# iqbal-lab-org/make_prg

Hardware: AMD Instinct MI355X
Metric: MSAs/sec (from_msa, whole node) on 30k-gene pan-genome (higher is better)
Workload: dtype u8 (+f64 KMeans)

## Files before the change

make_prg_amd/csrc/k_partition.inc:

```
MPRG_DEV bool col_is_nonmatch(const uint32_t *mask, int c) { return consensus_code(mask[c]) == 255; }

#define GR_ROWS 256
#ifndef GR_SEG
#define GR_SEG 512
#endif
#ifndef GR_BATCH
#define GR_BATCH 16
#endif
MPRG_DEV long long gr_items(long long S, long long n) { return ((S + GR_ROWS - 1) / GR_ROWS) * ((n + GR_SEG - 1) / GR_SEG); }
KERNEL(k_gap_runs, const uint8_t *arena, const int64_t *views, const int32_t *rowidx, const int32_t *work,
       const uint32_t *mask_all, uint32_t *maxrun_all, DsCount dc) {
  DS_GUARD(dc, 1);
  const int32_t *wk = work + 2 * (long long)BLOCK_ID;
  const ViewD d = load_view(views, wk[0]);
  const int n_chunks = (d.n_rows + GR_ROWS - 1) / GR_ROWS;
  const int r0 = (wk[1] % n_chunks) * GR_ROWS, cA = (wk[1] / n_chunks) * GR_SEG, cB = cA + GR_SEG < d.n_cols ? cA + GR_SEG : d.n_cols;
  const uint32_t *mask = mask_all + d.col_off;
  uint32_t *maxrun = maxrun_all + d.col_off;
  SHARED(int, has_gap, 1);
  ONE_THREAD { has_gap[0] = 0; }
  BARRIER();
  PAR_FOR(c, cB - cA) { if (mask[cA + c] & BIT_GAP) has_gap[0] = 1; }
  BARRIER();
  if (!has_gap[0]) return;
// ... 223 lines not shown
    int status = 0, cnt = 0, expect = 0, im = 0, in = 0;
    const int pure = (sh[4] || sh[5]) ? 0 : 2;
    while (im < nm || in < nn) {
      const bool takeM = in >= nn || (im < nm && Ms[2 * im] <= Ns[2 * in]);
      int s, e, type;
      if (takeM) { s = Ms[2 * im]; e = Ms[2 * im + 1]; type = pure; ++im; }
      else {
        s = Ns[2 * in]; e = Ns[2 * in + 1];
        const int ty = FAST ? ntype_s[in] : NTYPE(in);
        if (ty == 3) status |= 2;
        type = ty & 1;
        ++in;
      }
      if (s != expect || e < s || e >= n) { status |= 1; break; }
      ivw[3 * cnt] = s; ivw[3 * cnt + 1] = e; ivw[3 * cnt + 2] = type;
      ++cnt;
      expect = e + 1;
    }
    if (expect != n || cnt != nm + nn) status |= 1;
    sh[6] = cnt; sh[3] = status; sh[7] = cnt > 0 ? (ivw[2] & 1) : 0;
  }
  P_BAR(); KM_T(20);
#undef PUSH_M
#undef PUSH_N
#undef NONMATCH
#undef NTYPE
#undef PCELL
#undef PCELL8
#undef P_FOR
#undef P_BAR
#undef P_ONE
}

template <bool WV = false>
MPRG_DEV void pt_outputs(int v, int *sh, bool fast, const uint8_t *nmz_s, int32_t *iv, int32_t *n_iv_out, int32_t *status_out,
                         int32_t *view_out KM_TPARAM) {
  if ((WV ? wave_lane() : MPRG_TID) == 0) {
    const int cnt = sh[6], status = sh[3];
    n_iv_out[v] = cnt;
    status_out[v] = status;
    if (view_out) {
      int32_t *o = view_out + 8 * (long long)v;
      o[0] = cnt; o[1] = status; o[2] = sh[7];
      o[3] = (sh[0] ? 1 : 0) | ((sh[4] || sh[5]) ? 2 : 0);
      o[4] = 0; o[5] = 0; o[6] = 0; o[7] = 0;
    }
  }
  KM_T(22);
  if (fast) {
    const int32_t *src = (const int32_t *)nmz_s;
    for (int e = WV ? wave_lane() : MPRG_TID; e < 3 * sh[6]; e += WV ? WAVE : (int)blockDim.x) iv[e] = src[e];
  }
}
#define PK_PER_THREAD 32
KERNEL(k_pack_scan, int n_views_cap, const int32_t *n_iv, int32_t *view_out, int32_t *iv_count, DsCount dc) {
  const int n_views = (int)ds_n(dc, n_views_cap);
  SHARED(int, scratch, 17);
  int base = 0;
  for (int v0 = 0; v0 < n_views; v0 += N_THREADS * PK_PER_THREAD) {
    const int v = v0 + (int)threadIdx.x * PK_PER_THREAD;
    int c[PK_PER_THREAD], sum = 0;
#pragma unroll
    for (int q = 0; q < PK_PER_THREAD; ++q) { c[q] = v + q < n_views ? n_iv[v + q] : 0; sum += c[q]; }
    int tot;
    int run = base + block_scan_excl(sum, scratch, &tot);
#pragma unroll
    for (int q = 0; q < PK_PER_THREAD; ++q) { if (v + q < n_views) view_out[8 * (long long)(v + q) + 4] = run; run += c[q]; }
    base += tot;
  }
  ONE_THREAD { iv_count[0] = base; }
}
#define PK_THREADS 256
KERNEL(k_pack_copy, int n_views, const int64_t *views, const int32_t *iv_all, const int32_t *view_out, int32_t *iv_packed, DsCount dc) {
  const int v = BLOCK_ID * (PK_THREADS / WAVE) + wave_id();
  if (v >= ds_n(dc, n_views)) return;
  const int32_t *o = view_out + 8 * (long long)v;
  const int32_t *src = iv_all + 3 * views[(long long)v * VF + 8];
  int32_t *dst = iv_packed + 3 * (long long)o[4];
  for (int e = wave_lane(); e < 3 * o[0]; e += WAVE) dst[e] = src[e];
}

KERNEL(k_partition, const int32_t *view_list, const uint8_t *arena, const int64_t *views, const int32_t *rowidx,
       const uint32_t *mask_all, int L, uint32_t *maxrun_all, int32_t *stack_all, int32_t *ivflag_all, int32_t *iv_all,
       int32_t *n_iv_out, int32_t *status_out, int32_t *view_out, DsCount dc) {
  DS_GUARD(dc, 1);
  KM_T0();
  const int v = view_list ? view_list[BLOCK_ID] : BLOCK_ID;
  const ViewD d = load_view(views, v);
  const int n = d.n_cols;
  const uint32_t *mask = mask_all + d.col_off;
  uint32_t *maxrun = maxrun_all + d.col_off;
  SHARED(int32_t, stk_s, 4 * PT_STACK);
  __shared__ __attribute__((aligned(16))) uint8_t nmz_s[PT_COLS];
  SHARED(int32_t, ntype_s, PT_STACK);
  const bool fast = n / (L > 1 ? L - 1 : 1) + 4 <= PT_STACK && n <= PT_COLS;
  int32_t *flag_multi = ivflag_all + 2 * d.col_off;
  int32_t *ref_row = flag_multi + n;
  int32_t *iv = iv_all + 3 * d.col_off;
  SHARED(int, sh, 8);
  ONE_THREAD { sh[0] = 0; sh[1] = 0; sh[2] = 0; sh[3] = 0; sh[4] = 0; sh[5] = 0; sh[6] = 0; sh[7] = 0; }
  BARRIER();
  PAR_FOR(c, n) {
    const uint32_t m = mask[c];
    if (m & BIT_N) sh[4] = 1;
    if (m & BITS_IUPAC) sh[5] = 1;
    const uint32_t mm = m & ~BIT_N;
    const bool star = !(mm != 0 && (mm & (mm - 1)) == 0 && (mm & BITS_IUPAC) == 0 && mm != BIT_GAP);
    if (star) sh[0] = 1;
    if (fast) nmz_s[c] = star ? 1 : 0;
  }
  BARRIER(); KM_T(16);
  if (fast) pt_phases<true, false>(arena, d, rowidx, mask, L, maxrun, stack_all + 4 * d.col_off, flag_multi, ref_row, iv, stk_s,
                                   PT_STACK, nmz_s, PT_COLS, ntype_s, sh, nullptr, 0 KM_TARG);
  else pt_phases<false, false>(arena, d, rowidx, mask, L, maxrun, stack_all + 4 * d.col_off, flag_multi, ref_row, iv, stk_s,
                               PT_STACK, nmz_s, PT_COLS, ntype_s, sh, nullptr, 0 KM_TARG);
  pt_outputs(v, sh, fast, nmz_s, iv, n_iv_out, status_out, view_out KM_TARG);
  KM_T(21);
}

#define PF_ROWS 512
#define PF_COLS 1024
#define PF_CELLS 8192
#define PF_STACK 128
// ... 190 lines not shown
```

make_prg_amd/csrc/k_rows.inc:

```
MPRG_DEV uint64_t hash_mix(uint64_t x) {
  x ^= x >> 30; x *= 0xbf58476d1ce4e5b9ULL; x ^= x >> 27; x *= 0x94d049bb133111ebULL; x ^= x >> 31;
  return x;
}
#ifdef MPRG_TEST_WEAK_HASH
#define MPRG_HASH_MIX(x) 1ULL
#else
#define MPRG_HASH_MIX(x) hash_mix(x)
#endif
MPRG_DEV int u_pitch(int n_cols) { return (n_cols + 15) & ~15; }
MPRG_DEV uint64_t wave_sum_u64(uint64_t v) {
#pragma unroll
  for (int d = 32; d >= 1; d >>= 1) v += (uint64_t)__shfl_xor((unsigned long long)v, d);
  return v;
}

#define UG_ROWS 256
#define UG_WIDE 4096
#define UG_ROWS_WIDE 8
#define UG_BATCH 4
MPRG_DEV int ug_chunk_rows(long long n_cols) { return n_cols > UG_WIDE ? UG_ROWS_WIDE : UG_ROWS; }
MPRG_DEV long long ug_chunks(long long S, long long n_cols) { const int ch = ug_chunk_rows(n_cols); return (S + ch - 1) / ch; }
MPRG_DEV uint64_t hash_word(uint64_t w, unsigned pos) { return MPRG_HASH_MIX(w ^ ((uint64_t)(pos + 1) << 40)); }
#define DW_WAVES 4
#define DW_ROWS 64
#define DW_SLOTS 128
#define DW_COLS 64
MPRG_DEV bool dw_is_small(long long S, long long n) { return S >= 1 && S <= DW_ROWS && n >= 1 && n <= DW_COLS; }
MPRG_DEV void ug_hash_rows(const uint8_t *arena, const ViewD &d, const int32_t *rowidx, int r0, int chunk, int wv, int n_waves,
                           uint8_t *ucodes_all, uint64_t *hashes, int32_t *ulen_all, uint8_t *gcodes_all) {
  const int n = d.n_cols, S = d.n_rows;
  const int upitch = u_pitch(n);
  uint8_t *U = ucodes_all + d.aux0;
  uint64_t *hg = hashes + 2 * d.row_off + S;
  int32_t *ulen = ulen_all + d.row_off;
  const int lane = wave_lane();
  int G = WAVE;
  while (G > 8 && 4 * (G >> 1) >= n) G >>= 1;
  const int rows_per_wave = WAVE / G, gl = lane & (G - 1), sub = lane / G;
  for (int ib = r0 + wv * rows_per_wave; ib < r0 + chunk && ib < S; ib += n_waves * rows_per_wave) {
    const int i = ib + sub;
    const bool live = i < S && i < r0 + chunk;
    const uint8_t *src = arena + d.rm + (long long)(live ? view_row(d, rowidx, i) : 0) * d.pitchC + d.col0;
    uint8_t *dst = U + (long long)i * upitch;
    uint8_t *gdst = gcodes_all ? gcodes_all + d.aux0 + (long long)i * upitch : nullptr;
    uint64_t g = 0;
    int len = 0;
#define UG_STEP(w_, c0_) do {                                                                                                          \
      const int c = (c0_) + 4 * gl;                                                                                                    \
      uint32_t w = (w_);                                                                                                               \
      if (live && c < n) {                                                                                                             \
        if (c + 4 > n) {                                                          \
          const uint32_t keep = 0xffffffffu >> (8 * (c + 4 - n));                                                                      \
          w = (w & keep) | (0x04040404u & ~keep);                                                                                      \
        }                                                                                                                              \
        g += hash_word(w, (unsigned)c);                                                                                                \
        if (gdst) __builtin_memcpy(gdst + c, &w, 4);                        \
      }                                                                                                                                \
      const uint32_t v = w ^ 0x04040404u;                                                                       \
      const uint32_t gap = ~(((v & 0x7f7f7f7fu) + 0x7f7f7f7fu) | v) & 0x80808080u;                \
      const int kept = 4 - __popc(gap);                                                                                                \
      int incl = kept;                                                                \
      for (int dd = 1; dd < G; dd <<= 1) { const int y = __shfl_up(incl, dd, G); if (gl >= dd) incl += y; }                            \
      const int at = len + incl - kept;                                                                                                \
      if (live) {                                                                                                                      \
        if (kept == 4) __builtin_memcpy(dst + at, &w, 4);                                                                              \
        else if (kept) {                                                                                                               \
          int o = at;                                                                                                                  \
          _Pragma("unroll") for (int u = 0; u < 4; ++u) if (!((gap >> (8 * u + 7)) & 1u)) dst[o++] = (uint8_t)(w >> (8 * u));        \
        }                                                                                                                              \
      }                                                                                                                                \
      len += __shfl(incl, G - 1, G);                                                                                                   \
    } while (0)
    if (n <= 4 * G) {
      uint32_t w0 = 0x04040404u;
      if (live && 4 * gl < n) __builtin_memcpy(&w0, src + 4 * gl, 4);
      UG_STEP(w0, 0);
    } else {
      for (int cb = 0; cb < n; cb += UG_BATCH * 4 * G) {
        uint32_t wq[UG_BATCH];
#pragma unroll
        for (int q = 0; q < UG_BATCH; ++q) {
          const int c = cb + q * 4 * G + 4 * gl;
          wq[q] = 0x04040404u;
          if (live && c < n) __builtin_memcpy(&wq[q], src + c, 4);
        }
#pragma unroll
        for (int q = 0; q < UG_BATCH; ++q) {
          if (cb + q * 4 * G >= n) break;
          UG_STEP(wq[q], cb + q * 4 * G);
        }
      }
    }
#undef UG_STEP
    for (int dd = G >> 1; dd >= 1; dd >>= 1) g += (uint64_t)__shfl_xor((unsigned long long)g, dd, G);
    if (live && gl == 0) { hg[i] = g; ulen[i] = len; }
  }
}
KERNEL(k_ungap_hash, const uint8_t *arena, const int64_t *views, const int32_t *rowidx, const int32_t *work,
       uint8_t *ucodes_all, uint64_t *hashes, int32_t *ulen_all, uint8_t *gcodes_all, int wave_form, DsCount dc) {
  DS_GUARD(dc, 1);
  const int32_t *wk = work + 2 * (long long)BLOCK_ID;
  const ViewD d = load_view(views, wk[0]);
  if (wave_form && dw_is_small(d.n_rows, d.n_cols)) return;
  const int chunk = ug_chunk_rows(d.n_cols);
  ug_hash_rows(arena, d, rowidx, wk[1] * chunk, chunk, wave_id(), N_THREADS / WAVE, ucodes_all, hashes, ulen_all, gcodes_all);
}

MPRG_DEV void ug_hash_u_rows(const ViewD &d, int r0, int chunk, int wv, int n_waves, const uint8_t *ucodes_all, uint64_t *hashes,
                             const int32_t *ulen_all) {
  const int n = d.n_cols, S = d.n_rows, upitch = u_pitch(n);
  const uint8_t *U = ucodes_all + d.aux0;
  uint64_t *hu_w = hashes + 2 * d.row_off;
  const int32_t *ulen = ulen_all + d.row_off;
  const int lane = wave_lane();
  int G = WAVE;
  while (G > 4 && 8 * (G >> 1) >= n) G >>= 1;
  const int rows_per_wave = WAVE / G, gl = lane & (G - 1), sub = lane / G;
  for (int ib = r0 + wv * rows_per_wave; ib < r0 + chunk && ib < S; ib += n_waves * rows_per_wave) {
    const int i = ib + sub;
    const bool live = i < S && i < r0 + chunk;
    const int len = live ? ulen[i] : 0;
    const uint8_t *row = U + (long long)(live ? i : 0) * upitch;
    uint64_t a = 0;
    for (int p = 8 * gl; p < len; p += 8 * G) {
      uint64_t w = *(const uint64_t *)(row + p);
      if (p + 8 > len) w &= 0xffffffffffffffffULL >> (8 * (p + 8 - len));
      a += hash_word(w, (unsigned)p);
    }
    for (int dd = G >> 1; dd >= 1; dd >>= 1) a += (uint64_t)__shfl_xor((unsigned long long)a, dd, G);
    if (live && gl == 0) hu_w[i] = a;
  }
}
KERNEL(k_ungap_hash_u, const int64_t *views, const int32_t *work, const uint8_t *ucodes_all, uint64_t *hashes, const int32_t *ulen_all,
       int wave_form, DsCount dc) {
  DS_GUARD(dc, 1);
  const int32_t *wk = work + 2 * (long long)BLOCK_ID;
  const ViewD d = load_view(views, wk[0]);
  if (wave_form && dw_is_small(d.n_rows, d.n_cols)) return;
  const int chunk = ug_chunk_rows(d.n_cols);
  ug_hash_u_rows(d, wk[1] * chunk, chunk, wave_id(), N_THREADS / WAVE, ucodes_all, hashes, ulen_all);
}

#define DD_ROWS 512
#define DD_SLOTS 1024
#define DD_EMPTY 0xffffffffffffffffULL
MPRG_DEV bool dd_diff_u16(const uint8_t *U, int upitch, int i, int j, int p0, int len) {
  const uint4 x = *(const uint4 *)(U + (long long)i * upitch + p0), y = *(const uint4 *)(U + (long long)j * upitch + p0);
  unsigned m[4] = {x.x ^ y.x, x.y ^ y.y, x.z ^ y.z, x.w ^ y.w};
  const int valid = len - p0;
  if (valid >= 16) return (m[0] | m[1] | m[2] | m[3]) != 0;
  unsigned bad = 0;
#pragma unroll
  for (int w = 0; w < 4; ++w) {
    const int vb = valid - 4 * w;
    const unsigned keep = vb >= 4 ? 0xffffffffu : (vb <= 0 ? 0u : ((1u << (8 * vb)) - 1u));
    bad |= m[w] & keep;
  }
  return bad != 0;
}
KERNEL(k_dedupe_scan_big, const uint8_t *arena, const int64_t *views, const int32_t *rowidx, const int32_t *work,
       const uint8_t *ucodes_all, const uint64_t *hashes, const int32_t *ulen_all, int32_t *rep_u_all, int32_t *rep_g_all, DsCount dc) {
  DS_GUARD(dc, 1);
  const int32_t *wk = work + 2 * (long long)BLOCK_ID;
  const ViewD d = load_view(views, wk[0]);
  const int n = d.n_cols, S = d.n_rows, chunk = ug_chunk_rows(n), r0 = wk[1] * chunk, upitch = u_pitch(n);
  if (S <= DD_ROWS) return;
  const uint8_t *U = ucodes_all + d.aux0;
  const uint64_t *hu = hashes + 2 * d.row_off, *hg = hu + S;
  const int32_t *ulen = ulen_all + d.row_off;
  __shared__ uint64_t s_hu[DD_ROWS], s_hg[DD_ROWS];
  __shared__ int32_t s_len[DD_ROWS];
  __shared__ int32_t s_ru[UG_ROWS], s_rg[UG_ROWS];
  const int i_end = r0 + chunk < S ? r0 + chunk : S;
  const int G = N_THREADS / chunk > 0 ? N_THREADS / chunk : 1, ri_ = (int)threadIdx.x % chunk, cls = (int)threadIdx.x / chunk;
  const int i = r0 + ri_;
  const bool live = cls < G && i < i_end;
  if (threadIdx.x < UG_ROWS) { s_ru[threadIdx.x] = 0x7fffffff; s_rg[threadIdx.x] = 0x7fffffff; }
  const uint64_t a = live ? hu[i] : 0, g = live ? hg[i] : 0;
  const int len = live ? ulen[i] : 0;
  const uint8_t *ri = arena + d.rm + (long long)(live ? view_row(d, rowidx, i) : 0) * d.pitchC + d.col0;
  for (int c0 = 0; c0 < i_end - 1; c0 += DD_ROWS) {
    BARRIER();
    const bool done_u = s_ru[ri_] != 0x7fffffff, done_g = s_rg[ri_] != 0x7fffffff;
    PAR_FOR(t, DD_ROWS) { if (c0 + t < S) { s_hu[t] = hu[c0 + t]; s_hg[t] = hg[c0 + t]; s_len[t] = ulen[c0 + t]; } }
    BARRIER();
    if (!live || i <= c0) continue;
    const int j1 = (i < c0 + DD_ROWS ? i : c0 + DD_ROWS) - c0;
    if (!done_u) {
      for (int t0 = cls; t0 < j1;) {
        int hit = 0x7fffffff;
        for (int t = t0; t < j1 && hit == 0x7fffffff; t += 8 * G) {
#pragma unroll
          for (int q = 7; q >= 0; --q) { const int tq = t + q * G; if (tq < j1 && s_hu[tq] == a && s_len[tq] == len) hit = tq; }
        }
        if (hit == 0x7fffffff) break;
        bool bad = false;
        for (int p = 0; p < len && !bad; p += 16) bad = dd_diff_u16(U, upitch, i, c0 + hit, p, len);
// ... 13 lines not shown
        bool bad = false;
        for (int c = 0; c < n && !bad; ++c) bad = ri[c] != rj[c];
        if (!bad) { atomicMin(&s_rg[ri_], c0 + hit); break; }
        t0 = hit + G;
      }
    }
  }
  BARRIER();
  if (live && cls == 0) {
    rep_u_all[d.row_off + i] = s_ru[ri_] == 0x7fffffff ? i : s_ru[ri_];
    rep_g_all[d.row_off + i] = s_rg[ri_] == 0x7fffffff ? i : s_rg[ri_];
  }
}

#define DD_EXACT(HU, HG, LEN, RU, RG)                                                                                   \
  P_FOR(i, S) {                                                                                                       \
    int ru = (int)i;                                                                                                    \
    const int len = LEN[i];                                                                                             \
    const uint64_t a = HU[i];                                                                                           \
    for (int j = 0; j < (int)i; ++j) {                                                                                  \
      if (HU[j] != a || LEN[j] != len) continue;                                                                        \
      bool bad = false;                                                                                                 \
      for (int p = 0; p < len && !bad; p += 16) bad = dd_diff_u16(U, upitch, (int)i, j, p, len);                        \
      if (!bad) { ru = j; break; }                                                                                      \
    }                                                                                                                   \
    int rg = (int)i;                                                                                                    \
    const uint64_t g = HG[i];                                                                                           \
    const uint8_t *ri = arena + d.rm + (long long)view_row(d, rowidx, i) * d.pitchC + d.col0;                           \
    for (int j = 0; j < (int)i; ++j) {                                                                                  \
      if (HG[j] != g) continue;                                                                                         \
      const uint8_t *rj = arena + d.rm + (long long)view_row(d, rowidx, j) * d.pitchC + d.col0;                         \
      bool bad = false;                                                                                                 \
      for (int c = 0; c < n && !bad; ++c) bad = ri[c] != rj[c];                                                         \
      if (!bad) { rg = j; break; }                                                                                      \
    }                                                                                                                   \
    RU[i] = ru; RG[i] = rg;                                                                                             \
  }

template <int ROWS, int SLOTS> struct DdLds {
  unsigned long long t_key[SLOTS];
  uint64_t s_hu[ROWS], s_hg[ROWS];
  int t_min[SLOTS];
  int32_t s_len[ROWS], s_ru[ROWS], s_rg[ROWS];
  long long wsum[16];
  int scan_tmp[17];
  int refuted[1];
};
template <bool WV> MPRG_DEV int dd_scan_excl(int v, int *scratch, int *total) {
  if (!WV) return block_scan_excl(v, scratch, total);
  const int incl = wave_scan_incl(v);
  *total = __shfl(incl, WAVE - 1);
  return incl - v;
}
template <bool WV, int ROWS, int SLOTS>
MPRG_DEV void dd_view(const int q, const ViewD &d, const uint8_t *arena, const int32_t *rowidx, int kmer_size,
                      uint8_t *ucodes_all, const uint8_t *gcodes_all, uint64_t *hashes, int32_t *ulen_all, int32_t *rep_u_all, int32_t *rep_g_all,
                      int32_t *d_of_row_all, int32_t *s_of_row_all, int32_t *reps_pos_all, int32_t *reps_len_all,
                      int32_t *seqrow_all, int64_t *occ_off_all, int64_t *summary, DdLds<ROWS, SLOTS> &L) {
#define P_FOR(i_, n_) for (long long i_ = WV ? wave_lane() : MPRG_TID; i_ < (long long)(n_); i_ += WV ? WAVE : (int)blockDim.x)
#define P_BAR() do { if (WV) WAVE_SYNC(); else BARRIER(); } while (0)
#define P_ONE if ((WV ? wave_lane() : MPRG_TID) == 0)
  const int n = d.n_cols, S = d.n_rows;
  const int upitch = u_pitch(n);
  const uint8_t *U = ucodes_all + d.aux0;
  const uint64_t *hu = hashes + 2 * d.row_off, *hg = hu + S;
  int32_t *ulen = ulen_all + d.row_off, *rep_u = rep_u_all + d.row_off, *rep_g = rep_g_all + d.row_off;
  int32_t *dor = d_of_row_all + d.row_off, *sor = s_of_row_all + d.row_off;
  int32_t *rpos = reps_pos_all + d.row_off, *rlen = reps_len_all + d.row_off, *seqrow = seqrow_all + d.row_off;
  int64_t *occ = occ_off_all + d.row_off + q;
  unsigned long long *t_key = L.t_key;
  int *t_min = L.t_min;
  uint64_t *s_hu = L.s_hu, *s_hg = L.s_hg;
  int32_t *s_len = L.s_len, *s_ru = L.s_ru, *s_rg = L.s_rg;
  int *scan_tmp = L.scan_tmp, *refuted = L.refuted;
  const bool in_lds = S <= ROWS;
  int32_t *RU = in_lds ? s_ru : rep_u, *RG = in_lds ? s_rg : rep_g;
  if (in_lds) {
    P_FOR(i, S) { s_hu[i] = hu[i]; s_hg[i] = hg[i]; s_len[i] = ulen[i]; }
    P_ONE { refuted[0] = 0; }
    unsigned slots = 64;
    while ((int)slots < 2 * S) slots <<= 1;
    for (int pass = 0; pass < 2; ++pass) {
      P_FOR(s, slots) { t_key[s] = DD_EMPTY; t_min[s] = 0x7fffffff; }
      P_BAR();
      P_FOR(i, S) {
        unsigned long long key = pass == 0 ? hash_mix(s_hu[i] + (uint64_t)s_len[i]) : s_hg[i];
        if (key == DD_EMPTY) key = 0;
        unsigned s = (unsigned)(key >> 7) & (slots - 1);
        for (;;) {
          const unsigned long long old = atomicCAS(&t_key[s], (unsigned long long)DD_EMPTY, key);
          if (old == DD_EMPTY || old == key) { atomicMin(&t_min[s], (int)i); break; }
          s = (s + 1) & (slots - 1);
        }
      }
      P_BAR();
      P_FOR(i, S) {
        unsigned long long key = pass == 0 ? hash_mix(s_hu[i] + (uint64_t)s_len[i]) : s_hg[i];
        if (key == DD_EMPTY) key = 0;
        unsigned s = (unsigned)(key >> 7) & (slots - 1);
        while (t_key[s] != key) s = (s + 1) & (slots - 1);
        (pass == 0 ? s_ru : s_rg)[i] = t_min[s];
      }
      P_BAR();
    }
    {
      const int nblk = upitch / 16;
      P_FOR(e, (long long)S * nblk) {
        const int i = (int)((unsigned)e / (unsigned)nblk), p0 = (int)((unsigned)e % (unsigned)nblk) * 16;
        const int j = s_ru[i], len = s_len[i];
        if (j != i && j != s_rg[i] && p0 < len && (s_len[j] != len || dd_diff_u16(U, upitch, i, j, p0, len))) refuted[0] = 1;
      }
      if (gcodes_all) {
        const uint8_t *Gc = gcodes_all + d.aux0;
        P_FOR(e, (long long)S * nblk) {
          const int i = (int)((unsigned)e / (unsigned)nblk), p0 = (int)((unsigned)e % (unsigned)nblk) * 16;
          const int j = s_rg[i];
          if (j != i && p0 < n && dd_diff_u16(Gc, upitch, i, j, p0, n)) refuted[0] = 1;
        }
      }
      const int nw = (n + 3) >> 2;
      P_FOR(e, gcodes_all ? 0 : (long long)S * nw) {
        const int i = (int)((unsigned)e / (unsigned)nw), c = ((int)((unsigned)e % (unsigned)nw)) << 2;
        const int j = s_rg[i];
        if (j == i) continue;
        uint32_t x, y;
        __builtin_memcpy(&x, arena + d.rm + (long long)view_row(d, rowidx, i) * d.pitchC + d.col0 + c, 4);
        __builtin_memcpy(&y, arena + d.rm + (long long)view_row(d, rowidx, j) * d.pitchC + d.col0 + c, 4);
        const uint32_t keep = c + 4 > n ? 0xffffffffu >> (8 * (c + 4 - n)) : 0xffffffffu;
        if ((x ^ y) & keep) refuted[0] = 1;
      }
    }
    P_BAR();
    if (refuted[0]) {
      DD_EXACT(s_hu, s_hg, s_len, s_ru, s_rg)
      P_BAR();
    }
  }
  int base_u = 0, base_d = 0, base_s = 0, base_g = 0, base_t = 0;
  long long sumlen = 0;
  for (int c0 = 0; c0 < S; c0 += WV ? WAVE : N_THREADS) {
    const int i = c0 + (WV ? wave_lane() : (int)threadIdx.x);
    const bool live = i < S;
    const int len = live ? (in_lds ? s_len[i] : ulen[i]) : 0;
    const bool is_u = live && RU[i] == i, is_g = live && RG[i] == i;
    const bool is_long = is_u && len >= kmer_size, is_short = is_u && !is_long;
    int tot_p, tot_t;
    const int ip = dd_scan_excl<WV>((is_u ? 1 : 0) | (is_long ? 1 << 10 : 0) | (is_g ? 1 << 20 : 0), scan_tmp, &tot_p);
    const int iu = ip & 1023, id = (ip >> 10) & 1023, is = iu - id;
    const int tot_u = tot_p & 1023, tot_d = (tot_p >> 10) & 1023, tot_s = tot_u - tot_d, tot_g = (tot_p >> 20) & 1023;
    const int it = dd_scan_excl<WV>(is_long ? len - kmer_size + 1 : 0, scan_tmp, &tot_t);
    if (is_u) { rpos[base_u + iu] = i; rlen[base_u + iu] = len; sumlen += len; }
    if (is_long) { dor[i] = base_d + id; sor[i] = -1; seqrow[base_d + id] = i; occ[base_d + id + 1] = (long long)base_t + it + (len - kmer_size + 1); }
    if (is_short) { dor[i] = -1; sor[i] = base_s + is; }
    if (live && in_lds) { rep_u[i] = s_ru[i]; rep_g[i] = s_rg[i]; }
    base_u += tot_u; base_d += tot_d; base_s += tot_s; base_g += tot_g; base_t += tot_t;
  }
  {
    long long v = wave_scan_incl_ll(sumlen);
    long long *wsum = L.wsum;
    if (wave_lane() == WAVE - 1) wsum[WV ? 0 : wave_id()] = v;
    P_BAR();
    P_ONE {
      long long tot = 0;
      for (int w = 0; w < (WV ? 1 : N_THREADS / WAVE); ++w) tot += wsum[w];
      occ[0] = 0;
      int64_t *sm = summary + 8 * (long long)q;
      sm[0] = base_u; sm[1] = base_g; sm[2] = base_d; sm[3] = base_t; sm[4] = tot; sm[5] = base_s; sm[6] = 0; sm[7] = 0;
    }
  }
  P_BAR();
  __threadfence_block();
  if (WV) WAVE_SYNC_GLOBAL();
  P_FOR(i, S) {
    const int r = RU[i];
    if (r != (int)i) { dor[i] = dor[r]; sor[i] = sor[r]; }
  }
#undef P_FOR
#undef P_BAR
#undef P_ONE
}
KERNEL(k_ungap_dedupe, const uint8_t *arena, const int64_t *views, const int32_t *rowidx, int kmer_size,
       uint8_t *ucodes_all, const uint8_t *gcodes_all, uint64_t *hashes, int32_t *ulen_all, int32_t *rep_u_all, int32_t *rep_g_all,
       int32_t *d_of_row_all, int32_t *s_of_row_all, int32_t *reps_pos_all, int32_t *reps_len_all,
       int32_t *seqrow_all, int64_t *occ_off_all, int64_t *summary, int wave_form, DsCount dc) {
  DS_GUARD(dc, 1);
  const ViewD d = load_view(views, BLOCK_ID);
  if (wave_form && dw_is_small(d.n_rows, d.n_cols)) return;
  __shared__ DdLds<DD_ROWS, DD_SLOTS> L;
  dd_view<false, DD_ROWS, DD_SLOTS>(BLOCK_ID, d, arena, rowidx, kmer_size, ucodes_all, gcodes_all, hashes, ulen_all, rep_u_all, rep_g_all, d_of_row_all,
                                    s_of_row_all, reps_pos_all, reps_len_all, seqrow_all, occ_off_all, summary, L);
}
KERNEL(k_dedupe_wave, const uint8_t *arena, const int64_t *views, const int32_t *rowidx, int n_views, int kmer_size,
       uint8_t *ucodes_all, uint8_t *gcodes_all, uint64_t *hashes, int32_t *ulen_all, int32_t *rep_u_all, int32_t *rep_g_all,
       int32_t *d_of_row_all, int32_t *s_of_row_all, int32_t *reps_pos_all, int32_t *reps_len_all,
       int32_t *seqrow_all, int64_t *occ_off_all, int64_t *summary, DsCount dc) {
  const long long q = (long long)BLOCK_ID * DW_WAVES + wave_id();
  if (q >= ds_n(dc, n_views)) return;
  const ViewD d = load_view(views, (int)q);
  if (!dw_is_small(d.n_rows, d.n_cols)) return;
  __shared__ DdLds<DW_ROWS, DW_SLOTS> L_all[DW_WAVES];
  ug_hash_rows(arena, d, rowidx, 0, d.n_rows, 0, 1, ucodes_all, hashes, ulen_all, gcodes_all);
  WAVE_SYNC_GLOBAL();
  ug_hash_u_rows(d, 0, d.n_rows, 0, 1, ucodes_all, hashes, ulen_all);
  WAVE_SYNC_GLOBAL();
  dd_view<true, DW_ROWS, DW_SLOTS>((int)q, d, arena, rowidx, kmer_size, ucodes_all, gcodes_all, hashes, ulen_all, rep_u_all, rep_g_all, d_of_row_all,
                                   s_of_row_all, reps_pos_all, reps_len_all, seqrow_all, occ_off_all, summary, L_all[wave_id()]);
}
#undef DD_EXACT
```

make_prg_amd/csrc/mprg_api.hip:

```cpp
#include "mprg_platform.h"
#include "../../include/mprg.h"
#include <stdio.h>
#include <initializer_list>
#include <string.h>

#include "k_ingest.inc"
#include "k_columns.inc"
#include "k_partition.inc"
#include "k_rows.inc"
#include "k_kmer.inc"
#include "k_kmeans.inc"
#include "k_kmeans_lds.inc"
#include "k_cluster.inc"
#include "k_kloop.inc"
#include "k_emit.inc"
#include "k_forest.inc"
#include "k_align.inc"
#include "k_star.inc"
#include "k_refine.inc"
#include "k_prog.inc"
#include "host_encoders.inc"
#include "host_batch.inc"

static thread_local char g_err[512] = "";
static int fail(const char *what) { snprintf(g_err, sizeof g_err, "%s", what); return -1; }

static int check_launch(const char *name) {
  hipError_t e = hipGetLastError();
  if (e != hipSuccess) { snprintf(g_err, sizeof g_err, "%s: %s", name, hipGetErrorString(e)); return -2; }
  return 0;
}

#include "runtime_api.inc"

#define BLOCK_VIEW 256
#include <stdlib.h>
static int env_threads(const char *name, int dflt, int hi = 1024) {
  const char *e = getenv(name);
  const int v = e ? atoi(e) : dflt;
  return (v >= 64 && v <= hi && v % 64 == 0) ? v : dflt;
}
static const int g_pf_threads = env_threads("MPRG_PF_THREADS", BLOCK_VIEW);
static const int g_dd_threads = env_threads("MPRG_DD_THREADS", BLOCK_VIEW, 512);
static const int g_km_threads = env_threads("MPRG_KM_THREADS", 256);
static const int g_km_wide_threads = env_threads("MPRG_KM_WIDE_THREADS", 1024);
static const int g_kp_threads = env_threads("MPRG_KP_THREADS", 0);
static const int g_kp_tiled = [] { const char *e = getenv("MPRG_KP_TILED"); return (e && atoi(e) == 0) ? 0 : 1; }();
static const int g_kpw_split = [] { const char *e = getenv("MPRG_KPW_SPLIT"); return (e && atoi(e) == 0) ? 0 : 1; }();
static const int g_kms_threads = env_threads("MPRG_KMS_THREADS", 128, 128);
static const int g_kml_flags = [] { const char *e = getenv("MPRG_KML_FLAGS"); return e ? (atoi(e) & 0x7f) : 0; }();
static const int g_kml_threads[KML_CLASSES] = {env_threads("MPRG_KML_THREADS0", 128, 256), env_threads("MPRG_KML_THREADS1", 128, 256),
                                               env_threads("MPRG_KML_THREADS2", 256, 1024), env_threads("MPRG_KML_THREADS3", 256, 1024),
                                               env_threads("MPRG_KML_THREADS4", 512, 1024), env_threads("MPRG_KML_THREADS5", 1024, 1024)};
template <class K> static int kml_raise_lds(K kernel, bool *raised, const char *what) {
  if (*raised) return 0;
  if (hipFuncSetAttribute((const void *)kernel, hipFuncAttributeMaxDynamicSharedMemorySize, KML_C5) != hipSuccess) return fail(what);
  *raised = true;
  return 0;
}
static const int g_cf_one = [] { const char *e = getenv("MPRG_CF_ONE"); return (e && atoi(e) == 0) ? 0 : 1; }();
static const int g_pw_wave = [] { const char *e = getenv("MPRG_WAVE_VIEWS"); return (e && atoi(e) == 0) ? 0 : 1; }();

extern "C" {

#ifndef MPRG_BUILD_TAG
#define MPRG_BUILD_TAG "hip gfx950"
#endif
const char *mprg_version(void) { return "mprg 0.2 (" MPRG_BUILD_TAG ")"; }
const char *mprg_last_error(void) { return g_err; }

int mprg_device_cus(void) {
  int dev = 0; hipDeviceProp_t p;
  if (hipGetDevice(&dev) != hipSuccess || hipGetDeviceProperties(&p, dev) != hipSuccess) return fail("no HIP device");
  return p.multiProcessorCount;
}

int mprg_ingest(const uint8_t *raw, const int64_t *msa_table, int n_msas, int64_t n_tiles, const uint8_t *n_replacement,
                uint8_t *arena, int64_t arena_bytes, int32_t *status, void *stream) {
  if (n_msas <= 0) return 0;
  if (hipMemsetAsync(arena, 15, (size_t)arena_bytes, (hipStream_t)stream) != hipSuccess) return fail("memset");
  if (hipMemsetAsync(status, 0, sizeof(int32_t) * n_msas, (hipStream_t)stream) != hipSuccess) return fail("memset");
  if (n_tiles > 0) LAUNCH(k_ingest, n_tiles, 256, stream, raw, msa_table, n_msas, n_replacement, arena, status);
  return check_launch("k_ingest");
}

int mprg_column_residue_counts(const uint8_t *raw, const int64_t *table, const int32_t *work, int n_work, int32_t *out,
                               void *stream) {
  if (n_work <= 0) return 0;
  LAUNCH(k_column_residue_counts, n_work, 256, stream, raw, table, work, out);
  return check_launch("k_column_residue_counts");
}

static int d_column_masks(const uint8_t *arena, const int64_t *views, const int32_t *rowidx, const int32_t *work,
                          int n_items, int rows_per_chunk, uint32_t *out_mask, void *stream, DsCount dc) {
  if (n_items <= 0) return 0;
  if (rows_per_chunk <= 0) return fail("rows_per_chunk must be positive");
  LAUNCH(k_column_masks, n_items, CM_THREADS, stream, arena, views, rowidx, work, rows_per_chunk, out_mask, dc);
  return check_launch("k_column_masks");
}
int mprg_column_masks(const uint8_t *arena, const int64_t *views, const int32_t *rowidx, const int32_t *work,
                      int n_items, int rows_per_chunk, uint32_t *out_mask, void *stream) {
  return d_column_masks(arena, views, rowidx, work, n_items, rows_per_chunk, out_mask, stream, DS_HOST);
}

int mprg_compact_columns(const uint8_t *arena, const int64_t *views, const int32_t *rowidx, const int32_t *work, int n_items,
                         int rows_per_chunk, const uint32_t *mask, uint8_t *out, const int64_t *out_off, int32_t *kept, void *stream) {
  if (n_items <= 0) return 0;
  if (rows_per_chunk <= 0) return fail("rows_per_chunk must be positive");
  LAUNCH(k_compact_columns, n_items, CC_THREADS, stream, arena, views, rowidx, work, rows_per_chunk, mask, out, out_off, kept);
  return check_launch("k_compact_columns");
}

static int d_partition(const uint8_t *arena, const int64_t *views, const int32_t *rowidx, int n_views,
                       const uint32_t *mask, int min_match_length, const int32_t *work_rows, int n_work_rows,
                       uint32_t *maxrun, int32_t *stack, int32_t *ivflag, int32_t *iv, int32_t *n_iv, int32_t *status,
                       int32_t *view_out, int32_t *iv_packed, int32_t *iv_count, const int32_t *fused_list, int n_fused,
                       const int32_t *other_list, int n_other, void *stream, DsCount dc_views, DsCount dc_rows, DsCount dc_fused,
                       DsCount dc_other);
int mprg_partition(const uint8_t *arena, const int64_t *views, const int32_t *rowidx, int n_views,
                   const uint32_t *mask, int min_match_length, const int32_t *work_rows, int n_work_rows,
                   uint32_t *maxrun, int32_t *stack, int32_t *ivflag, int32_t *iv, int32_t *n_iv, int32_t *status,
                   int32_t *view_out, int32_t *iv_packed, int32_t *iv_count, const int32_t *fused_list, int n_fused,
                   const int32_t *other_list, int n_other, void *stream) {
  return d_partition(arena, views, rowidx, n_views, mask, min_match_length, work_rows, n_work_rows, maxrun, stack, ivflag, iv, n_iv, status,
                     view_out, iv_packed, iv_count, fused_list, n_fused, other_list, n_other, stream, DS_HOST, DS_HOST, DS_HOST, DS_HOST);
}
static int d_partition(const uint8_t *arena, const int64_t *views, const int32_t *rowidx, int n_views,
                       const uint32_t *mask, int min_match_length, const int32_t *work_rows, int n_work_rows,
                       uint32_t *maxrun, int32_t *stack, int32_t *ivflag, int32_t *iv, int32_t *n_iv, int32_t *status,
                       int32_t *view_out, int32_t *iv_packed, int32_t *iv_count, const int32_t *fused_list, int n_fused,
                       const int32_t *other_list, int n_other, void *stream, DsCount dc_views, DsCount dc_rows, DsCount dc_fused,
                       DsCount dc_other) {
  if (n_views <= 0) return 0;
  if (!fused_list && !other_list) { n_fused = 0; n_other = n_views; }
  else if (n_fused < 0 || n_other < 0 || (!dc_views.ds && n_fused + n_other != n_views)) return fail("mprg_partition: the two view lists must cover the views");
  else if ((n_fused > 0 && !fused_list) || (n_other > 0 && !other_list)) return fail("mprg_partition: a view list is missing");
  if (min_match_length < 1) return fail("mprg_partition: min_match_length must be positive");
  if (n_work_rows > 0) LAUNCH(k_gap_runs, n_work_rows, GR_ROWS, stream, arena, views, rowidx, work_rows, mask, maxrun, dc_rows);
  if (n_other > 0)
    LAUNCH(k_partition, n_other, BLOCK_VIEW, stream, other_list, arena, views, rowidx, mask, min_match_length, maxrun, stack,
           ivflag, iv, n_iv, status, view_out, dc_other);
  if (n_fused > 0) {
    if (g_pw_wave) LAUNCH(k_partition_wave, (n_fused + PW_WAVES - 1) / PW_WAVES, PW_WAVES * WAVE, stream, fused_list, arena, views, rowidx,
                          min_match_length, iv, n_iv, status, view_out, n_fused, dc_fused);
    LAUNCH(k_partition_fused, n_fused, g_pf_threads, stream, fused_list, arena, views, rowidx, min_match_length, iv, n_iv, status,
           view_out, g_pw_wave, dc_fused);
  }
  if (view_out) {
    if (!iv_packed || !iv_count) return fail("mprg_partition: view_out needs iv_packed and iv_count");
    LAUNCH(k_pack_scan, 1, 1024, stream, n_views, n_iv, view_out, iv_count, dc_views);
    LAUNCH(k_pack_copy, (n_views + PK_THREADS / WAVE - 1) / (PK_THREADS / WAVE), PK_THREADS, stream, n_views, views, iv, view_out,
           iv_packed, dc_views);
  }
  return check_launch("k_partition");
}

static int d_ungap_dedupe(const uint8_t *arena, const int64_t *views, const int32_t *rowidx, int n_views, int kmer_size,
                          const int32_t *work_rows, int n_work_rows, uint8_t *ucodes, uint64_t *hashes, int32_t *ulen,
                          int32_t *rep_u, int32_t *rep_g, int32_t *d_of_row, int32_t *s_of_row, int32_t *reps_pos,
                          int32_t *reps_len, int32_t *seqrow, int64_t *occ_off, int64_t *summary, uint8_t *gcodes, void *stream,
                          DsCount dc_views, DsCount dc_rows, long long max_rows = 0) {
  if (n_views <= 0) return 0;
  if (g_pw_wave)
    LAUNCH(k_dedupe_wave, (n_views + DW_WAVES - 1) / DW_WAVES, DW_WAVES * WAVE, stream, arena, views, rowidx, n_views, kmer_size, ucodes, gcodes, hashes,
           ulen, rep_u, rep_g, d_of_row, s_of_row, reps_pos, reps_len, seqrow, occ_off, summary, dc_views);
  if (n_work_rows > 0) {
    LAUNCH(k_ungap_hash, n_work_rows, UG_ROWS, stream, arena, views, rowidx, work_rows, ucodes, hashes, ulen, gcodes, g_pw_wave, dc_rows);
    LAUNCH(k_ungap_hash_u, n_work_rows, UG_ROWS, stream, views, work_rows, (const uint8_t *)ucodes, hashes, (const int32_t *)ulen, g_pw_wave, dc_rows);
    if (max_rows > 0 ? max_rows > DD_ROWS : (dc_rows.ds != nullptr || n_work_rows > n_views))
      LAUNCH(k_dedupe_scan_big, n_work_rows, UG_ROWS, stream, arena, views, rowidx, work_rows, (const uint8_t *)ucodes, (const uint64_t *)hashes,
             (const int32_t *)ulen, rep_u, rep_g, dc_rows);
  }
  LAUNCH(k_ungap_dedupe, n_views, g_dd_threads, stream, arena, views, rowidx, kmer_size, ucodes, (const uint8_t *)gcodes, hashes, ulen, rep_u, rep_g,
         d_of_row, s_of_row, reps_pos, reps_len, seqrow, occ_off, summary, g_pw_wave, dc_views);
  return check_launch("k_ungap_dedupe");
}
int mprg_ungap_dedupe(const uint8_t *arena, const int64_t *views, const int32_t *rowidx, int n_views, int kmer_size,
                      const int32_t *work_rows, int n_work_rows, uint8_t *ucodes, uint64_t *hashes, int32_t *ulen,
                      int32_t *rep_u, int32_t *rep_g, int32_t *d_of_row, int32_t *s_of_row, int32_t *reps_pos,
                      int32_t *reps_len, int32_t *seqrow, int64_t *occ_off, int64_t *summary, uint8_t *gcodes, void *stream) {
  return d_ungap_dedupe(arena, views, rowidx, n_views, kmer_size, work_rows, n_work_rows, ucodes, hashes, ulen, rep_u, rep_g, d_of_row, s_of_row,
                        reps_pos, reps_len, seqrow, occ_off, summary, gcodes, stream, DS_HOST, DS_HOST);
}

int mprg_kmer_dictionary(const int64_t *views, const int64_t *prob, int n_probs, int kmer_size,
                         const uint8_t *ucodes, const int32_t *ulen, const int32_t *seqrow, int64_t *occ_off,
                         uint8_t *table, uint8_t *first_flag, int32_t *out_V, void *stream) {
  (void)ulen;
  if (n_probs <= 0) return 0;
  if (kmer_size < 1) return fail("k-mer size must be positive");
  LAUNCH(k_kmer_dictionary, n_probs, KD_THREADS, stream, views, prob, kmer_size, ucodes, seqrow, (const int64_t *)occ_off, table,
         first_flag, out_V, DS_HOST);
  return check_launch("k_kmer_dictionary");
}

int mprg_kmer_dictionary_parts(const int64_t *views, const int64_t *prob, int n_probs, int kmer_size, const uint8_t *ucodes,
                               const int32_t *ulen, const int32_t *seqrow, int64_t *occ_off, uint8_t *table, uint8_t *first_flag,
                               int32_t *out_V, int parts, int32_t *part_counts, void *stream) {
  (void)ulen;
  if (n_probs <= 0) return 0;
  if (kmer_size < 1 || kmer_size > KMER_PACKED_MAX) return fail("mprg_kmer_dictionary_parts: k-mer sizes 1..16 (packed keys)");
  if (parts < 1 || parts > 1024 || !part_counts) return fail("mprg_kmer_dictionary_parts: parts must be 1..1024, part_counts given");
  LAUNCH2(k_kmer_dict_clear, n_probs, parts, 256, stream, views, prob, ucodes, seqrow, (const int64_t *)occ_off, table);
  LAUNCH2(k_kmer_dict_insert, n_probs, parts, 256, stream, views, prob, kmer_size, ucodes, seqrow, (const int64_t *)occ_off, table);
  LAUNCH2(k_kmer_dict_ids, n_probs, parts, 256, stream, views, prob, kmer_size, ucodes, seqrow, (const int64_t *)occ_off, table, first_flag,
          part_counts, out_V, 0);
  LAUNCH2(k_kmer_dict_ids, n_probs, parts, 256, stream, views, prob, kmer_size, ucodes, seqrow, (const int64_t *)occ_off, table, first_flag,
          part_counts, out_V, 1);
  return check_launch("k_kmer_dict_ids");
}
int mprg_kmer_counts_parts(const int64_t *views, const int64_t *prob, int n_probs, int kmer_size, const uint8_t *ucodes,
                           const int32_t *ulen, const int32_t *seqrow, const int64_t *occ_off, const uint8_t *table,
                           double *xcounts, int parts, void *stream) {
  (void)ulen;
  if (n_probs <= 0) return 0;
  if (kmer_size < 1) return fail("k-mer size must be positive");
  if (parts < 1 || parts > 1024) return fail("mprg_kmer_counts_parts: parts must be 1..1024");
  LAUNCH2(k_kmer_counts, n_probs, parts, 512, stream, views, prob, kmer_size, ucodes, seqrow, occ_off, table, xcounts, DS_HOST);
  return check_launch("k_kmer_counts");
}
int mprg_kmer_counts(const int64_t *views, const int64_t *prob, int n_probs, int kmer_size, const uint8_t *ucodes,
                     const int32_t *ulen, const int32_t *seqrow, const int64_t *occ_off, const uint8_t *table,
                     double *xcounts, void *stream) {
  return mprg_kmer_counts_parts(views, prob, n_probs, kmer_size, ucodes, ulen, seqrow, occ_off, table, xcounts, 1, stream);
}

int64_t mprg_kmeans_workspace_doubles(int64_t D, int64_t V, int k_max, int n_restart_slots) {
// ... 867 lines not shown
```

Baseline: 132,300.

## Fuse row ungap/hash with dedupe for narrow views and parallelize pack scan

After: 134,800 (median of 6 runs). 1.02x the previous value.

```diff
diff --git a/make_prg_amd/csrc/k_partition.inc b/make_prg_amd/csrc/k_partition.inc
--- a/make_prg_amd/csrc/k_partition.inc
+++ b/make_prg_amd/csrc/k_partition.inc
@@ -299,23 +299,27 @@
     for (int e = WV ? wave_lane() : MPRG_TID; e < 3 * sh[6]; e += WV ? WAVE : (int)blockDim.x) iv[e] = src[e];
   }
 }
-#define PK_PER_THREAD 32
+#define PK_SCAN_THREADS 1024
+#define PK_SCAN_PER_THREAD 8
+#define PK_VIEWS (PK_SCAN_THREADS * PK_SCAN_PER_THREAD)
 KERNEL(k_pack_scan, int n_views_cap, const int32_t *n_iv, int32_t *view_out, int32_t *iv_count, DsCount dc) {
   const int n_views = (int)ds_n(dc, n_views_cap);
+  const int v0 = BLOCK_ID * PK_VIEWS;
+  if (BLOCK_ID > 0 && v0 >= n_views) return;
   SHARED(int, scratch, 17);
-  int base = 0;
-  for (int v0 = 0; v0 < n_views; v0 += N_THREADS * PK_PER_THREAD) {
-    const int v = v0 + (int)threadIdx.x * PK_PER_THREAD;
-    int c[PK_PER_THREAD], sum = 0;
-#pragma unroll
-    for (int q = 0; q < PK_PER_THREAD; ++q) { c[q] = v + q < n_views ? n_iv[v + q] : 0; sum += c[q]; }
-    int tot;
-    int run = base + block_scan_excl(sum, scratch, &tot);
-#pragma unroll
-    for (int q = 0; q < PK_PER_THREAD; ++q) { if (v + q < n_views) view_out[8 * (long long)(v + q) + 4] = run; run += c[q]; }
-    base += tot;
-  }
-  ONE_THREAD { iv_count[0] = base; }
+  int part = 0;
+  for (int u = (int)threadIdx.x; u < v0; u += PK_SCAN_THREADS) part += n_iv[u];
+  int base;
+  block_scan_excl(part, scratch, &base);
+  const int v = v0 + (int)threadIdx.x * PK_SCAN_PER_THREAD;
+  int c[PK_SCAN_PER_THREAD], sum = 0;
+#pragma unroll
+  for (int q = 0; q < PK_SCAN_PER_THREAD; ++q) { c[q] = v + q < n_views ? n_iv[v + q] : 0; sum += c[q]; }
+  int tot;
+  int run = base + block_scan_excl(sum, scratch, &tot);
+#pragma unroll
+  for (int q = 0; q < PK_SCAN_PER_THREAD; ++q) { if (v + q < n_views) view_out[8 * (long long)(v + q) + 4] = run; run += c[q]; }
+  if (v0 + PK_VIEWS >= n_views) ONE_THREAD { iv_count[0] = base + tot; }
 }
 #define PK_THREADS 256
 KERNEL(k_pack_copy, int n_views, const int64_t *views, const int32_t *iv_all, const int32_t *view_out, int32_t *iv_packed, DsCount dc) {
diff --git a/make_prg_amd/csrc/k_rows.inc b/make_prg_amd/csrc/k_rows.inc
--- a/make_prg_amd/csrc/k_rows.inc
+++ b/make_prg_amd/csrc/k_rows.inc
@@ -26,6 +26,16 @@
 #define DW_SLOTS 128
 #define DW_COLS 64
 MPRG_DEV bool dw_is_small(long long S, long long n) { return S >= 1 && S <= DW_ROWS && n >= 1 && n <= DW_COLS; }
+#define DD_ROWS 512
+#define DD_SLOTS 1024
+#define RV_COLS 64
+#define RV_ROWS_S 128
+#define RV_SLOTS_S 256
+#define RF_WAVE 1
+#define RF_ROWS 2
+MPRG_DEV bool rv_is_narrow(long long S, long long n) { return n >= 1 && n <= RV_COLS && S >= 1 && S <= DD_ROWS; }
+MPRG_DEV bool rv_takes(int form, long long S, long long n) { return (form & RF_ROWS) && rv_is_narrow(S, n) && !((form & RF_WAVE) && dw_is_small(S, n)); }
+MPRG_DEV bool rows_elsewhere(int form, long long S, long long n) { return ((form & RF_WAVE) && dw_is_small(S, n)) || rv_takes(form, S, n); }
 MPRG_DEV void ug_hash_rows(const uint8_t *arena, const ViewD &d, const int32_t *rowidx, int r0, int chunk, int wv, int n_waves,
                            uint8_t *ucodes_all, uint64_t *hashes, int32_t *ulen_all, uint8_t *gcodes_all) {
   const int n = d.n_cols, S = d.n_rows;
@@ -97,11 +107,11 @@
   }
 }
 KERNEL(k_ungap_hash, const uint8_t *arena, const int64_t *views, const int32_t *rowidx, const int32_t *work,
-       uint8_t *ucodes_all, uint64_t *hashes, int32_t *ulen_all, uint8_t *gcodes_all, int wave_form, DsCount dc) {
+       uint8_t *ucodes_all, uint64_t *hashes, int32_t *ulen_all, uint8_t *gcodes_all, int form, DsCount dc) {
   DS_GUARD(dc, 1);
   const int32_t *wk = work + 2 * (long long)BLOCK_ID;
   const ViewD d = load_view(views, wk[0]);
-  if (wave_form && dw_is_small(d.n_rows, d.n_cols)) return;
+  if (rows_elsewhere(form, d.n_rows, d.n_cols)) return;
   const int chunk = ug_chunk_rows(d.n_cols);
   ug_hash_rows(arena, d, rowidx, wk[1] * chunk, chunk, wave_id(), N_THREADS / WAVE, ucodes_all, hashes, ulen_all, gcodes_all);
 }
@@ -132,17 +142,15 @@
   }
 }
 KERNEL(k_ungap_hash_u, const int64_t *views, const int32_t *work, const uint8_t *ucodes_all, uint64_t *hashes, const int32_t *ulen_all,
-       int wave_form, DsCount dc) {
+       int form, DsCount dc) {
   DS_GUARD(dc, 1);
   const int32_t *wk = work + 2 * (long long)BLOCK_ID;
   const ViewD d = load_view(views, wk[0]);
-  if (wave_form && dw_is_small(d.n_rows, d.n_cols)) return;
+  if (rows_elsewhere(form, d.n_rows, d.n_cols)) return;
   const int chunk = ug_chunk_rows(d.n_cols);
   ug_hash_u_rows(d, wk[1] * chunk, chunk, wave_id(), N_THREADS / WAVE, ucodes_all, hashes, ulen_all);
 }
 
-#define DD_ROWS 512
-#define DD_SLOTS 1024
 #define DD_EMPTY 0xffffffffffffffffULL
 MPRG_DEV bool dd_diff_u16(const uint8_t *U, int upitch, int i, int j, int p0, int len) {
   const uint4 x = *(const uint4 *)(U + (long long)i * upitch + p0), y = *(const uint4 *)(U + (long long)j * upitch + p0);
@@ -262,7 +270,7 @@
   *total = __shfl(incl, WAVE - 1);
   return incl - v;
 }
-template <bool WV, int ROWS, int SLOTS>
+template <bool WV, int ROWS, int SLOTS, bool LOADED = false>
 MPRG_DEV void dd_view(const int q, const ViewD &d, const uint8_t *arena, const int32_t *rowidx, int kmer_size,
                       uint8_t *ucodes_all, const uint8_t *gcodes_all, uint64_t *hashes, int32_t *ulen_all, int32_t *rep_u_all, int32_t *rep_g_all,
                       int32_t *d_of_row_all, int32_t *s_of_row_all, int32_t *reps_pos_all, int32_t *reps_len_all,
@@ -286,7 +294,7 @@
   const bool in_lds = S <= ROWS;
   int32_t *RU = in_lds ? s_ru : rep_u, *RG = in_lds ? s_rg : rep_g;
   if (in_lds) {
-    P_FOR(i, S) { s_hu[i] = hu[i]; s_hg[i] = hg[i]; s_len[i] = ulen[i]; }
+    if (!LOADED) P_FOR(i, S) { s_hu[i] = hu[i]; s_hg[i] = hg[i]; s_len[i] = ulen[i]; }
     P_ONE { refuted[0] = 0; }
     unsigned slots = 64;
     while ((int)slots < 2 * S) slots <<= 1;
@@ -392,14 +400,98 @@
 KERNEL(k_ungap_dedupe, const uint8_t *arena, const int64_t *views, const int32_t *rowidx, int kmer_size,
        uint8_t *ucodes_all, const uint8_t *gcodes_all, uint64_t *hashes, int32_t *ulen_all, int32_t *rep_u_all, int32_t *rep_g_all,
        int32_t *d_of_row_all, int32_t *s_of_row_all, int32_t *reps_pos_all, int32_t *reps_len_all,
-       int32_t *seqrow_all, int64_t *occ_off_all, int64_t *summary, int wave_form, DsCount dc) {
+       int32_t *seqrow_all, int64_t *occ_off_all, int64_t *summary, int form, DsCount dc) {
   DS_GUARD(dc, 1);
   const ViewD d = load_view(views, BLOCK_ID);
-  if (wave_form && dw_is_small(d.n_rows, d.n_cols)) return;
+  if (rows_elsewhere(form, d.n_rows, d.n_cols)) return;
   __shared__ DdLds<DD_ROWS, DD_SLOTS> L;
   dd_view<false, DD_ROWS, DD_SLOTS>(BLOCK_ID, d, arena, rowidx, kmer_size, ucodes_all, gcodes_all, hashes, ulen_all, rep_u_all, rep_g_all, d_of_row_all,
                                     s_of_row_all, reps_pos_all, reps_len_all, seqrow_all, occ_off_all, summary, L);
 }
+#define RV_BATCH 8
+template <bool WV>
+MPRG_DEV void rv_rows(const uint8_t *arena, const ViewD &d, const int32_t *rowidx, uint8_t *ucodes_all, uint64_t *hashes,
+                      int32_t *ulen_all, uint8_t *gcodes_all, uint64_t *s_hu, uint64_t *s_hg, int32_t *s_len) {
+  const int n = d.n_cols, S = d.n_rows, upitch = u_pitch(n);
+  uint64_t *hu = hashes + 2 * d.row_off, *hg = hu + S;
+  int32_t *ulen = ulen_all + d.row_off;
+  for (long long i = WV ? wave_lane() : MPRG_TID; i < S; i += WV ? WAVE : (int)blockDim.x) {
+    const uint8_t *src = arena + d.rm + (long long)view_row(d, rowidx, i) * d.pitchC + d.col0;
+    uint8_t *dst = ucodes_all + d.aux0 + i * upitch;
+    uint8_t *gdst = gcodes_all ? gcodes_all + d.aux0 + i * upitch : nullptr;
+    uint64_t g = 0, a = 0, acc = 0;
+    int fill = 0, p = 0;
+    for (int cb = 0; cb < n; cb += 4 * RV_BATCH) {
+      uint32_t wq[RV_BATCH];
+#pragma unroll
+      for (int q = 0; q < RV_BATCH; ++q) {
+        const int c = cb + 4 * q;
+        wq[q] = 0x04040404u;
+        if (c < n) __builtin_memcpy(&wq[q], src + c, 4);
+      }
+#pragma unroll
+      for (int q = 0; q < RV_BATCH; ++q) {
+        const int c = cb + 4 * q;
+        if (c >= n) break;
+        uint32_t w = wq[q];
+        if (c + 4 > n) {
+          const uint32_t keep = 0xffffffffu >> (8 * (c + 4 - n));
+          w = (w & keep) | (0x04040404u & ~keep);
+        }
+        g += hash_word(w, (unsigned)c);
+        if (gdst) __builtin_memcpy(gdst + c, &w, 4);
+        const uint32_t v = w ^ 0x04040404u;
+        const uint32_t gap = ~(((v & 0x7f7f7f7fu) + 0x7f7f7f7fu) | v) & 0x80808080u;
+        uint32_t kw = w;
+        int k = 4;
+        if (gap) {
+          kw = 0; k = 0;
+#pragma unroll
+          for (int u = 0; u < 4; ++u) {
+            const bool keep = !((gap >> (8 * u + 7)) & 1u);
+            kw |= keep ? ((w >> (8 * u)) & 0xffu) << (8 * k) : 0u;
+            k += keep ? 1 : 0;
+          }
+        }
+        acc |= (uint64_t)kw << (8 * fill);
+        fill += k;
+        if (fill >= 8) {
+          __builtin_memcpy(dst + p, &acc, 8);
+          a += hash_word(acc, (unsigned)p);
+          p += 8; fill -= 8;
+          acc = (uint64_t)kw >> (8 * (k - fill));
+        }
+      }
+    }
+    if (fill > 0) {
+      __builtin_memcpy(dst + p, &acc, 8);
+      a += hash_word(acc, (unsigned)p);
+    }
+    const int len = p + fill;
+    hu[i] = a; hg[i] = g; ulen[i] = len;
+    s_hu[i] = a; s_hg[i] = g; s_len[i] = len;
+  }
+}
+#define RV_PARAMS const uint8_t *arena, const int64_t *views, const int32_t *rowidx, int kmer_size,                              \
+       uint8_t *ucodes_all, uint8_t *gcodes_all, uint64_t *hashes, int32_t *ulen_all, int32_t *rep_u_all, int32_t *rep_g_all, \
+       int32_t *d_of_row_all, int32_t *s_of_row_all, int32_t *reps_pos_all, int32_t *reps_len_all,                            \
+       int32_t *seqrow_all, int64_t *occ_off_all, int64_t *summary, int form, DsCount dc
+#define RV_BODY(ROWS_, SLOTS_, mine_) do {                                                                                            \
+    DS_GUARD(dc, 1);                                                                                                                  \
+    const ViewD d = load_view(views, BLOCK_ID);                                                                                       \
+    if (!rv_takes(form, d.n_rows, d.n_cols) || !(mine_)) return;                                                                      \
+    __shared__ DdLds<ROWS_, SLOTS_> L;                                                                                                \
+    rv_rows<false>(arena, d, rowidx, ucodes_all, hashes, ulen_all, gcodes_all, L.s_hu, L.s_hg, L.s_len);                              \
+    __threadfence_block();                 \
+    BARRIER();                                                                                                                        \
+    dd_view<false, ROWS_, SLOTS_, true>(BLOCK_ID, d, arena, rowidx, kmer_size, ucodes_all, gcodes_all, hashes, ulen_all, rep_u_all,   \
+                                        rep_g_all, d_of_row_all, s_of_row_all, reps_pos_all, reps_len_all, seqrow_all, occ_off_all,   \
+                                        summary, L);                                                                                  \
+  } while (0)
+KERNEL(k_rows_narrow, RV_PARAMS) { RV_BODY(DD_ROWS, DD_SLOTS, d.n_rows > RV_ROWS_S); }
+KERNEL(k_rows_narrow_s, RV_PARAMS) { RV_BODY(RV_ROWS_S, RV_SLOTS_S, d.n_rows <= RV_ROWS_S); }
+#undef RV_BODY
+#undef RV_PARAMS
 KERNEL(k_dedupe_wave, const uint8_t *arena, const int64_t *views, const int32_t *rowidx, int n_views, int kmer_size,
        uint8_t *ucodes_all, uint8_t *gcodes_all, uint64_t *hashes, int32_t *ulen_all, int32_t *rep_u_all, int32_t *rep_g_all,
        int32_t *d_of_row_all, int32_t *s_of_row_all, int32_t *reps_pos_all, int32_t *reps_len_all,
@@ -416,4 +508,20 @@
   dd_view<true, DW_ROWS, DW_SLOTS>((int)q, d, arena, rowidx, kmer_size, ucodes_all, gcodes_all, hashes, ulen_all, rep_u_all, rep_g_all, d_of_row_all,
                                    s_of_row_all, reps_pos_all, reps_len_all, seqrow_all, occ_off_all, summary, L_all[wave_id()]);
 }
+KERNEL(k_rows_wave, const uint8_t *arena, const int64_t *views, const int32_t *rowidx, int n_views, int kmer_size,
+       uint8_t *ucodes_all, uint8_t *gcodes_all, uint64_t *hashes, int32_t *ulen_all, int32_t *rep_u_all, int32_t *rep_g_all,
+       int32_t *d_of_row_all, int32_t *s_of_row_all, int32_t *reps_pos_all, int32_t *reps_len_all,
+       int32_t *seqrow_all, int64_t *occ_off_all, int64_t *summary, DsCount dc) {
+  const long long q = (long long)BLOCK_ID * DW_WAVES + wave_id();
+  if (q >= ds_n(dc, n_views)) return;
+  const ViewD d = load_view(views, (int)q);
+  if (!dw_is_small(d.n_rows, d.n_cols)) return;
+  __shared__ DdLds<DW_ROWS, DW_SLOTS> L_all[DW_WAVES];
+  DdLds<DW_ROWS, DW_SLOTS> &L = L_all[wave_id()];
+  rv_rows<true>(arena, d, rowidx, ucodes_all, hashes, ulen_all, gcodes_all, L.s_hu, L.s_hg, L.s_len);
+  WAVE_SYNC_GLOBAL();
+  WAVE_SYNC();
+  dd_view<true, DW_ROWS, DW_SLOTS, true>((int)q, d, arena, rowidx, kmer_size, ucodes_all, gcodes_all, hashes, ulen_all, rep_u_all, rep_g_all, d_of_row_all,
+                                         s_of_row_all, reps_pos_all, reps_len_all, seqrow_all, occ_off_all, summary, L);
+}
 #undef DD_EXACT
diff --git a/make_prg_amd/csrc/mprg_api.hip b/make_prg_amd/csrc/mprg_api.hip
--- a/make_prg_amd/csrc/mprg_api.hip
+++ b/make_prg_amd/csrc/mprg_api.hip
@@ -60,6 +60,9 @@
 }
 static const int g_cf_one = [] { const char *e = getenv("MPRG_CF_ONE"); return (e && atoi(e) == 0) ? 0 : 1; }();
 static const int g_pw_wave = [] { const char *e = getenv("MPRG_WAVE_VIEWS"); return (e && atoi(e) == 0) ? 0 : 1; }();
+static const int g_row_views = [] { const char *e = getenv("MPRG_ROW_VIEWS"); return (e && atoi(e) == 0) ? 0 : 1; }();
+#define RV_THREADS 128
+#define RV_THREADS_S 64
 
 extern "C" {
 
@@ -148,7 +151,7 @@
   }
   if (view_out) {
     if (!iv_packed || !iv_count) return fail("mprg_partition: view_out needs iv_packed and iv_count");
-    LAUNCH(k_pack_scan, 1, 1024, stream, n_views, n_iv, view_out, iv_count, dc_views);
+    LAUNCH(k_pack_scan, (n_views + PK_VIEWS - 1) / PK_VIEWS, PK_SCAN_THREADS, stream, n_views, n_iv, view_out, iv_count, dc_views);
     LAUNCH(k_pack_copy, (n_views + PK_THREADS / WAVE - 1) / (PK_THREADS / WAVE), PK_THREADS, stream, n_views, views, iv, view_out,
            iv_packed, dc_views);
   }
@@ -161,18 +164,28 @@
                           int32_t *reps_len, int32_t *seqrow, int64_t *occ_off, int64_t *summary, uint8_t *gcodes, void *stream,
                           DsCount dc_views, DsCount dc_rows, long long max_rows = 0) {
   if (n_views <= 0) return 0;
-  if (g_pw_wave)
+  const int form = (g_pw_wave ? RF_WAVE : 0) | (g_row_views ? RF_ROWS : 0);
+  if (g_pw_wave && g_row_views)
+    LAUNCH(k_rows_wave, (n_views + DW_WAVES - 1) / DW_WAVES, DW_WAVES * WAVE, stream, arena, views, rowidx, n_views, kmer_size, ucodes, gcodes, hashes,
+           ulen, rep_u, rep_g, d_of_row, s_of_row, reps_pos, reps_len, seqrow, occ_off, summary, dc_views);
+  else if (g_pw_wave)
     LAUNCH(k_dedupe_wave, (n_views + DW_WAVES - 1) / DW_WAVES, DW_WAVES * WAVE, stream, arena, views, rowidx, n_views, kmer_size, ucodes, gcodes, hashes,
            ulen, rep_u, rep_g, d_of_row, s_of_row, reps_pos, reps_len, seqrow, occ_off, summary, dc_views);
+  if (g_row_views) {
+    LAUNCH(k_rows_narrow, n_views, RV_THREADS, stream, arena, views, rowidx, kmer_size, ucodes, gcodes, hashes, ulen, rep_u, rep_g, d_of_row, s_of_row,
+           reps_pos, reps_len, seqrow, occ_off, summary, form, dc_views);
+    LAUNCH(k_rows_narrow_s, n_views, RV_THREADS_S, stream, arena, views, rowidx, kmer_size, ucodes, gcodes, hashes, ulen, rep_u, rep_g, d_of_row, s_of_row,
+           reps_pos, reps_len, seqrow, occ_off, summary, form, dc_views);
+  }
   if (n_work_rows > 0) {
-    LAUNCH(k_ungap_hash, n_work_rows, UG_ROWS, stream, arena, views, rowidx, work_rows, ucodes, hashes, ulen, gcodes, g_pw_wave, dc_rows);
-    LAUNCH(k_ungap_hash_u, n_work_rows, UG_ROWS, stream, views, work_rows, (const uint8_t *)ucodes, hashes, (const int32_t *)ulen, g_pw_wave, dc_rows);
+    LAUNCH(k_ungap_hash, n_work_rows, UG_ROWS, stream, arena, views, rowidx, work_rows, ucodes, hashes, ulen, gcodes, form, dc_rows);
+    LAUNCH(k_ungap_hash_u, n_work_rows, UG_ROWS, stream, views, work_rows, (const uint8_t *)ucodes, hashes, (const int32_t *)ulen, form, dc_rows);
     if (max_rows > 0 ? max_rows > DD_ROWS : (dc_rows.ds != nullptr || n_work_rows > n_views))
       LAUNCH(k_dedupe_scan_big, n_work_rows, UG_ROWS, stream, arena, views, rowidx, work_rows, (const uint8_t *)ucodes, (const uint64_t *)hashes,
              (const int32_t *)ulen, rep_u, rep_g, dc_rows);
   }
   LAUNCH(k_ungap_dedupe, n_views, g_dd_threads, stream, arena, views, rowidx, kmer_size, ucodes, (const uint8_t *)gcodes, hashes, ulen, rep_u, rep_g,
-         d_of_row, s_of_row, reps_pos, reps_len, seqrow, occ_off, summary, g_pw_wave, dc_views);
+         d_of_row, s_of_row, reps_pos, reps_len, seqrow, occ_off, summary, form, dc_views);
   return check_launch("k_ungap_dedupe");
 }
 int mprg_ungap_dedupe(const uint8_t *arena, const int64_t *views, const int32_t *rowidx, int n_views, int kmer_size,
```
